# jhidalgocarrio/slam-localization

Hardware: NVIDIA B200
Metric: filter-steps/sec (predict+update) (higher is better)
Workload: dtype f64

## Files before the change

### slam-localization_b200/csrc/slb_api.cu

```cuda
#include <cstdio>
#include <cstdlib>
#include <cstring>
#include <atomic>
#include <new>

#include <dlfcn.h>
#include <nccl.h>

#include "slb_internal.h"
#include "slb_math.cuh"

namespace slb {

static thread_local char g_err[512] = "";
static std::atomic<int64_t> g_launches{0};

int set_error(int code, const char *what, cudaError_t ce) {
    if (ce != cudaSuccess)
        snprintf(g_err, sizeof(g_err), "%s: %s", what, cudaGetErrorString(ce));
    else
        snprintf(g_err, sizeof(g_err), "%s", what);
    return code;
}
void count_launch(int n) { g_launches.fetch_add(n, std::memory_order_relaxed); }
// ... 21 lines not shown
    const int c = e - r * (r + 1) / 2;
    soa[(size_t)e * stride + B0 + i] = dense[(size_t)i * N * N + r * N + c];
}
__global__ void soa_to_dense_P(const double *soa, double *dense, int B0, int cnt, int N, int stride) {
    const int64_t t = (int64_t)blockIdx.x * blockDim.x + threadIdx.x;
    if (t >= (int64_t)cnt * N * N) return;
    const int i = (int)(t / (N * N)), rc = (int)(t - (int64_t)i * N * N);
    int r = rc / N, c = rc - r * N;
    if (c > r) { const int x = r; r = c; c = x; }
    dense[t] = soa[(size_t)(r * (r + 1) / 2 + c) * stride + B0 + i];
}
__global__ void aos_to_rec_mu(const double *aos, double *rec, int B0, int cnt, int QD, int qstride) {
    const int t = blockIdx.x * blockDim.x + threadIdx.x;
    if (t >= cnt * QD) return;
    const int i = t / QD, c = t - i * QD;
    rec[(size_t)(B0 + i) * qstride + c] = aos[t];
}
__global__ void rec_to_aos_mu(const double *rec, double *aos, int B0, int cnt, int QD, int qstride, int off = 0) {
    const int t = blockIdx.x * blockDim.x + threadIdx.x;
    if (t >= cnt * QD) return;
    const int i = t / QD, c = t - i * QD;
    aos[t] = rec[(size_t)(B0 + i) * qstride + off + c];
}
__global__ void dense_to_rec_P(const double *dense, double *rec, int B0, int cnt, int N, int pstride) {
    const int64_t t = (int64_t)blockIdx.x * blockDim.x + threadIdx.x;
    if (t >= (int64_t)cnt * N * N) return;
    const int i = (int)(t / (N * N)), rc = (int)(t - (int64_t)i * N * N);
    const int r = rc / N, c = rc - r * N;
    if (c <= r) rec[(size_t)(B0 + i) * pstride + r * (r + 1) / 2 + c] = dense[t];
}
__global__ void rec_to_dense_P(const double *rec, double *dense, int B0, int cnt, int N, int pstride) {
    const int64_t t = (int64_t)blockIdx.x * blockDim.x + threadIdx.x;
    if (t >= (int64_t)cnt * N * N) return;
    const int i = (int)(t / (N * N)), rc = (int)(t - (int64_t)i * N * N);
    int r = rc / N, c = rc - r * N;
    if (c > r) { const int x = r; r = c; c = x; }
    dense[t] = rec[(size_t)(B0 + i) * pstride + r * (r + 1) / 2 + c];
}

__global__ void replicate_soa(double *a, int rows, int stride, int B, int count) {
    const int64_t t = (int64_t)blockIdx.x * blockDim.x + threadIdx.x;
    if (t >= (int64_t)rows * B) return;
    const int r = (int)(t / B), i = (int)(t - (int64_t)r * B);
    if (i >= count) a[(size_t)r * stride + i] = a[(size_t)r * stride + i % count];
}
__global__ void replicate_rec(double *a, int per, int B, int count) {
    const int64_t t = (int64_t)blockIdx.x * blockDim.x + threadIdx.x;
    if (t >= (int64_t)per * B) return;
    const int i = (int)(t / per), e = (int)(t - (int64_t)i * per);
    if (i >= count) a[(size_t)i * per + e] = a[(size_t)(i % count) * per + e];
}

__global__ void status_count(const int32_t *st, int B, unsigned long long *counts) {
    unsigned long long c[SLB_NSTATUS];
#pragma unroll
    for (int b = 0; b < SLB_NSTATUS; ++b) c[b] = 0;
    for (int i = blockIdx.x * blockDim.x + threadIdx.x; i < B; i += gridDim.x * blockDim.x) {
        const int s = st[i];
#pragma unroll
        for (int b = 0; b < SLB_NSTATUS; ++b) c[b] += (s >> b) & 1;
// ... 218 lines not shown
    if (!h || offset < 0 || count < 1 || offset + count > h->QD)
        return set_error(SLB_ERR_INVALID, "slb_set_output_slice: the slice must lie inside the q-vector");
    h->out_off = offset;
    h->out_len = count;
    return SLB_OK;
}
int slb_dof(slb_handle h) { return h ? h->N : SLB_ERR_INVALID; }
int slb_qdim(slb_handle h) { return h ? h->QD : SLB_ERR_INVALID; }

int slb_device_ptr(slb_handle h, int field, void **dev) {
    if (!h || !dev) return set_error(SLB_ERR_INVALID, "slb_device_ptr: null argument");
    switch (field) {
        case SLB_FIELD_MU: *dev = h->mu; return SLB_OK;
        case SLB_FIELD_P: *dev = h->P; return SLB_OK;
        case SLB_FIELD_STATUS: *dev = h->status; return SLB_OK;
        case SLB_FIELD_OUTLIERS: *dev = h->outliers; return SLB_OK;
    }
    return set_error(SLB_ERR_INVALID, "slb_device_ptr: unknown field");
}

static int transfer(slb_handle h, int field, void *host, size_t count, cudaStream_t s, bool up) {
    if (!h || !host) return set_error(SLB_ERR_INVALID, "slb_upload/download: null argument");
    DeviceGuard guard(h->cfg.device);
    const bool soa = h->cfg.kind == SLB_KIND_UKF;
    if (field == SLB_FIELD_STATUS || field == SLB_FIELD_OUTLIERS) {
        if (up) return set_error(SLB_ERR_INVALID, "slb_upload: status fields are read-only");
        if (count != (size_t)h->B) return set_error(SLB_ERR_INVALID, "slb_download: count must equal batch");
        SLB_CUDA(cudaMemcpyAsync(host, field == SLB_FIELD_STATUS ? h->status : h->outliers, (size_t)h->B * 4,
                                 cudaMemcpyDeviceToHost, s));
        SLB_CUDA(cudaStreamSynchronize(s));
        return SLB_OK;
    }
    size_t per;
    if (field == SLB_FIELD_MU) per = h->QD;
    else if (field == SLB_FIELD_P) per = (size_t)h->N * h->N;
    else return set_error(SLB_ERR_INVALID, "slb_upload/download: unknown field");
    if (count == 0 || count % per != 0 || count > per * h->B)
        return set_error(SLB_ERR_INVALID, "slb_upload/download: count must be k * per-instance size, 1 <= k <= batch");
    const int nin = (int)(count / per);
    const int chunk = (int)(h->stage_bytes / (per * 8));
    double *hp = (double *)host;
    for (int b0 = 0; b0 < nin; b0 += chunk) {
        const int cnt = (nin - b0) < chunk ? (nin - b0) : chunk;
        const size_t bytes = (size_t)cnt * per * 8;
        const int64_t work = (int64_t)cnt * (field == SLB_FIELD_MU ? h->QD : (up && soa ? h->NP : h->N * h->N));
        const int tpb = 256;
        const int grid = (int)((work + tpb - 1) / tpb);
        if (up) {
            SLB_CUDA(cudaMemcpyAsync(h->stage, hp + (size_t)b0 * per, bytes, cudaMemcpyHostToDevice, s));
            if (field == SLB_FIELD_MU) {
                if (soa) aos_to_soa_mu<<<grid, tpb, 0, s>>>(h->stage, h->mu, b0, cnt, h->QD, h->stride);
                else aos_to_rec_mu<<<grid, tpb, 0, s>>>(h->stage, h->mu, b0, cnt, h->QD, h->qstride);
            } else {
                if (soa) dense_to_soa_P<<<grid, tpb, 0, s>>>(h->stage, h->P, b0, cnt, h->N, h->stride);
                else dense_to_rec_P<<<grid, tpb, 0, s>>>(h->stage, h->P, b0, cnt, h->N, h->pstride);
            }
            count_launch();
            SLB_CUDA(cudaGetLastError());
        } else {
            if (field == SLB_FIELD_MU) {
                if (soa) soa_to_aos_mu<<<grid, tpb, 0, s>>>(h->mu, h->stage, b0, cnt, h->QD, h->stride);
                else rec_to_aos_mu<<<grid, tpb, 0, s>>>(h->mu, h->stage, b0, cnt, h->QD, h->qstride);
            } else {
                if (soa) soa_to_dense_P<<<grid, tpb, 0, s>>>(h->P, h->stage, b0, cnt, h->N, h->stride);
                else rec_to_dense_P<<<grid, tpb, 0, s>>>(h->P, h->stage, b0, cnt, h->N, h->pstride);
            }
            count_launch();
            SLB_CUDA(cudaGetLastError());
            SLB_CUDA(cudaMemcpyAsync(hp + (size_t)b0 * per, h->stage, bytes, cudaMemcpyDeviceToHost, s));
        }
        SLB_CUDA(cudaStreamSynchronize(s));
    }
    return SLB_OK;
}

int slb_upload(slb_handle h, int field, const void *host, size_t count, void *stream) {
    return transfer(h, field, const_cast<void *>(host), count, S(stream), true);
}
int slb_download(slb_handle h, int field, void *host, size_t count, void *stream) {
    return transfer(h, field, host, count, S(stream), false);
}

int slb_replicate(slb_handle h, int count, void *stream) {
    if (!h || count <= 0 || count > h->B) return set_error(SLB_ERR_INVALID, "slb_replicate: bad count");
    DeviceGuard guard(h->cfg.device);
    cudaStream_t s = S(stream);
    if (count == h->B) return SLB_OK;
    const int tpb = 256;
// ... 572 lines not shown
```

### slam-localization_b200/csrc/slb_check.cu

```cuda
#include "slb_internal.h"
#include "slb_math.cuh"

namespace slbd {

struct ChkLayout {
    int nblk;
    unsigned long long so3mask;
    int nfeat;
    int N, QD, NP, pstride, qstride;
};

SLB_DEV double warp_max(double v) {
#pragma unroll
    for (int o = 16; o > 0; o >>= 1) v = fmax(v, __shfl_xor_sync(0xffffffffu, v, o));
    return v;
}

__global__ void __launch_bounds__(32) check_sigma_points_kernel(const double *mu, const double *P, int B, ChkLayout l,
                                                                int32_t *flags, double *diff) {
    extern __shared__ double sm[];
    const int lane = threadIdx.x;
    const int N = l.N, QD = l.QD, NP = l.NP, NS = 2 * N + 1;
    double *Lp = sm, *Pa = Lp + NP, *D = Pa + NP, *mus = D + 32 * N, *ref = mus + QD, *md = ref + QD;
    for (int inst = blockIdx.x; inst < B; inst += gridDim.x) {
        const double *Pg = P + (size_t)inst * l.pstride, *mug = mu + (size_t)inst * l.qstride;
        __syncwarp();
        for (int e = lane; e < NP; e += 32) { Lp[e] = Pg[e]; Pa[e] = 0.0; }
        for (int e = lane; e < QD; e += 32) { mus[e] = mug[e]; ref[e] = mug[e]; }
        __syncwarp();
        bool ok = true;
        for (int k = 0; k < N && ok; ++k) {
            const double dkk = Lp[tri(k, k)];
            ok = dkk > 0.0;
            if (!ok) break;
            const double s = sqrt(dkk), inv = 1.0 / s;
            __syncwarp();
            for (int i = k + lane; i < N; i += 32) Lp[tri(i, k)] = i == k ? s : Lp[tri(i, k)] * inv;
            __syncwarp();
            for (int i = k + 1 + lane; i < N; i += 32) {
                const double lik = Lp[tri(i, k)];
                for (int j = k + 1; j <= i; ++j) Lp[tri(i, j)] = fma(-lik, Lp[tri(j, k)], Lp[tri(i, j)]);
            }
            __syncwarp();
        }
        if (!ok) {
            if (lane == 0) {
                flags[inst] = 4;
                if (diff) { diff[2 * (size_t)inst] = 0.0; diff[2 * (size_t)inst + 1] = 0.0; }
            }
            continue;
// ... 67 lines not shown
                        } else {
                            for (int c = 0; c < 3; ++c) ref[o + c] += md[3 * b + c];
                        }
                    }
                    o += so3 ? 4 : 3;
                }
                for (int f = lane; f < l.nfeat; f += 32) ref[o + f] += md[3 * l.nblk + f];
            }
            __syncwarp();
        } while (sqrt(nrm2) > 1e-6 && ++it < 10000);
        for (int s0 = 0; s0 < NS; s0 += 32) {
            __syncwarp();
            deviation(s0 + lane);
            __syncwarp();
            for (int i = 0; i < N; ++i)
                for (int j = lane; j <= i; j += 32) {
                    double a = 0.0;
                    for (int t = 0; t < 32; ++t) a = fma(D[t * N + i], D[t * N + j], a);
                    Pa[tri(i, j)] += 0.5 * a;
                }
        }
        __syncwarp();
        double dP = 0.0;
        for (int e = lane; e < NP; e += 32) dP = fmax(dP, fabs(Pa[e] - Pg[e]));
        dP = warp_max(dP);
        double dm = 0.0;
        {
            int o = 0;
            for (int b = 0; b < l.nblk; ++b) {
                const bool so3 = (l.so3mask >> b) & 1ull;
                if (b % 32 == lane) {
                    if (so3) {
                        const double q[4] = {mus[o], mus[o + 1], mus[o + 2], mus[o + 3]};
                        const double r[4] = {ref[o], ref[o + 1], ref[o + 2], ref[o + 3]};
                        double t[4], w[3];
                        quat_cmul(q, r, t);
                        so3_log(t, w);
                        for (int c = 0; c < 3; ++c) dm = fmax(dm, fabs(w[c]));
                    } else {
                        for (int c = 0; c < 3; ++c) dm = fmax(dm, fabs(ref[o + c] - mus[o + c]));
                    }
                }
                o += so3 ? 4 : 3;
            }
            for (int f = lane; f < l.nfeat; f += 32) dm = fmax(dm, fabs(ref[o + f] - mus[o + f]));
        }
        dm = warp_max(dm);
        if (lane == 0) {
            flags[inst] = (!(dP <= 1e-6) ? 1 : 0) | (!(dm <= 1e-12) ? 2 : 0);
            if (diff) { diff[2 * (size_t)inst] = dP; diff[2 * (size_t)inst + 1] = dm; }
        }
    }
}

}

namespace slb {

int launch_check_sigma_points(const slb_batch_s *h, int32_t *flags, double *diff, cudaStream_t s) {
    slbd::ChkLayout l;
    l.N = h->N; l.QD = h->QD; l.NP = h->NP; l.pstride = h->pstride; l.qstride = h->qstride;
    l.so3mask = 0;
    if (h->cfg.kind == SLB_KIND_USCKF) {
        l.nblk = 12; l.nfeat = h->cfg.nk + h->cfg.nl;
        l.so3mask = (1ull << 1) | (1ull << 5) | (1ull << 9);
    } else if (h->cfg.kind == SLB_KIND_MSCKF) {
        l.nblk = 4 + 2 * h->cfg.nclones; l.nfeat = 0;
        l.so3mask = 1ull << 1;
        for (int j = 0; j < h->cfg.nclones; ++j) l.so3mask |= 1ull << (4 + 2 * j + 1);
    } else {
        return set_error(SLB_ERR_INVALID, "slb_check_sigma_points: Usckf / Msckf batches only (the reference's ukfom::ukf has no checkSigmaPoints)");
    }
    const size_t smem = ((size_t)2 * l.NP + 32 * l.N + 2 * l.QD + l.N) * sizeof(double);
    SLB_CUDA(cudaFuncSetAttribute(slbd::check_sigma_points_kernel, cudaFuncAttributeMaxDynamicSharedMemorySize, (int)smem));
    int grid = h->B < 148 * 3 * 8 ? h->B : 148 * 3 * 8;
    slbd::check_sigma_points_kernel<<<grid, 32, smem, s>>>(h->mu, h->P, h->B, l, flags, diff);
    count_launch();
    SLB_CUDA(cudaGetLastError());
    return SLB_OK;
}

}
```

### slam-localization_b200/csrc/slb_math.cuh

```cuda
#pragma once
#include <cuda_runtime.h>
#include <stdint.h>

namespace slbd {

#define SLB_DEV __device__ __forceinline__
#define SLB_HD __host__ __device__ __forceinline__

template <int NB_, unsigned MASK_>
struct Layout {
    static constexpr int NB = NB_;
    static constexpr unsigned MASK = MASK_;
    static constexpr int N = 3 * NB_;
    static constexpr int NP = N * (N + 1) / 2;
    SLB_HD static constexpr bool so3(int b) { return (MASK_ >> b) & 1u; }
    SLB_HD static constexpr int qoff(int b) {
        int o = 0;
        for (int i = 0; i < b; ++i) o += ((MASK_ >> i) & 1u) ? 4 : 3;
        return o;
    }
    static constexpr int QD = qoff(NB_);
};
typedef Layout<2, 0x2> LayPose6;
typedef Layout<3, 0x2> LayMtk9;
typedef Layout<4, 0x2> LayState12;

SLB_HD constexpr int tri(int i, int j) { return i * (i + 1) / 2 + j; }

SLB_DEV double rcp_fast(double w) {
    double r;
    asm("rcp.approx.ftz.f64 %0, %1;" : "=d"(r) : "d"(w));
    double e = fma(-w, r, 1.0);
    r = fma(r, e, r);
    e = fma(-w, r, 1.0);
    r = fma(r, e, r);
    return r;
}
SLB_DEV void sqrt_rsqrt(double x, double &s, double &rs) {
    double y;
    asm("rsqrt.approx.ftz.f64 %0, %1;" : "=d"(y) : "d"(x));
    double e = fma(-(x * y), y, 1.0);
    y = fma(0.5 * y, e, y);
    e = fma(-(x * y), y, 1.0);
    y = fma(0.5 * y, e, y);
    double r = x * y;
    r = fma(fma(-r, r, x), 0.5 * y, r);
    s = r;
    rs = y;
}

// ... 167 lines not shown
```

### slam-localization_b200/csrc/slb_predict12.cuh

```cuda
#pragma once
#include "slb_internal.h"
#include "slb_models.cuh"

namespace slbd {

constexpr unsigned FULL = 0xffffffffu;
SLB_DEV double warp_sum(double v) {
#pragma unroll
    for (int o = 16; o > 0; o >>= 1) v += __shfl_xor_sync(FULL, v, o);
    return v;
}
SLB_DEV double bcast(double v, int src) { return __shfl_sync(FULL, v, src); }

template <int N_>
struct CycCfg {
    static constexpr int N = N_;
    static constexpr int RT = (N_ + 3) / 4;
    static constexpr int CT = (N_ + 7) / 8;
    SLB_HD static constexpr int cb(int k) { return k * N_ - k * (k - 1) / 2; }
    SLB_HD static constexpr bool exists(int r, int c) { return 4 * r < N_ && 8 * c < N_ && 4 * r + 3 >= 8 * c; }
    SLB_HD static constexpr bool live(int k, int r, int c) { return exists(r, c) && 8 * c + 7 > k && 4 * r + 3 > k; }
    SLB_HD static constexpr bool row_live(int k, int r) {
        for (int c = 0; c < CT; ++c)
            if (live(k, r, c)) return true;
// ... 60 lines not shown
}
SLB_DEV void bulk_g2s(void *dst, const void *src, unsigned bytes, uint64_t *bar) {
    asm volatile("cp.async.bulk.shared::cluster.global.mbarrier::complete_tx::bytes [%0], [%1], %2, [%3];\n" ::"r"(saddr(dst)),
                 "l"(src), "r"(bytes), "r"(saddr(bar))
                 : "memory");
}
SLB_DEV void mbar_wait(uint64_t *bar, unsigned parity) {
    unsigned done = 0;
    while (!done) {
        asm volatile(
            "{\n .reg .pred p;\n mbarrier.try_wait.parity.shared::cta.b64 p, [%1], %2;\n selp.u32 %0, 1, 0, p;\n}\n"
            : "=r"(done)
            : "r"(saddr(bar)), "r"(parity)
            : "memory");
    }
}

SLB_DEV void dmma884(double &d0, double &d1, double a, double b) {
    asm volatile("mma.sync.aligned.m8n8k4.row.col.f64.f64.f64.f64 {%0,%1}, {%2}, {%3}, {%0,%1};\n"
                 : "+d"(d0), "+d"(d1)
                 : "d"(a), "d"(b));
}

constexpr int PRED_PR = 366;
constexpr int PRED_PF = 28 * 12;
constexpr int PRED_DS = 20;
constexpr int PRED_LS = 78 + 16;
constexpr int PRED_SM = PRED_PR + PRED_PF + PRED_LS + 28 * PRED_DS + 144 + 12 * PRED_DS + 16 + 2;
static_assert(16 * PRED_SM * 8 <= 227 * 1024, "two CTAs of 8 warps per SM");
SLB_DEV void pred_cp_async8(double *smem_dst, const double *gsrc) {
    asm volatile("cp.async.ca.shared.global [%0], [%1], 8;\n" ::"r"(saddr(smem_dst)), "l"(gsrc) : "memory");
}
SLB_DEV void pred_cp_async_wait_all() { asm volatile("cp.async.commit_group;\n cp.async.wait_group 0;\n" ::: "memory"); }

template <int PM, int WPB, int ROW0, int MU0, bool CROSS>
__global__ void __launch_bounds__(WPB * 32, 2) predict12_kernel(slb::FilterArgs a) {
    typedef LayState12 L;
    typedef CycCfg<12> C;
    extern __shared__ __align__(16) double smem[];
    const int lane = threadIdx.x & 31, w = threadIdx.x >> 5;
    const int inst = blockIdx.x * WPB + w;
    if (inst >= a.B) return;
    double *Pr = smem + (size_t)w * PRED_SM, *Pf = Pr + PRED_PR, *Ls = Pf + PRED_PF, *D = Ls + PRED_LS, *W = D + 28 * PRED_DS,
           *Fk = W + 144, *rsd = Fk + 12 * PRED_DS;
    const int nf = CROSS ? a.nk + a.nl : 0;
    constexpr int T0 = ROW0 * (ROW0 + 1) / 2, T1 = (ROW0 + 12) * (ROW0 + 13) / 2, SPAN = T1 - T0;
    static_assert(SPAN <= PRED_PR, "row span");
    double *Pg = a.P + (size_t)inst * a.pstride;
    double *mug = a.mu + (size_t)inst * a.qstride;
    auto PR = [&](int r, int c) -> double & { return Pr[tri(ROW0 + r, c) - T0]; };
    const int a_ = lane & 3, b_ = lane >> 2;

    static_assert((T0 * 8) % 16 == 0 && (SPAN * 8) % 16 == 0 && PRED_SM % 2 == 0, "bulk copy needs 16-byte alignment");
    uint64_t *bar = reinterpret_cast<uint64_t *>(rsd + 16);
    if (lane == 0) {
        mbar_init(bar, 1);
        mbar_expect_tx(bar, SPAN * 8);
        bulk_g2s(Pr, Pg + T0, SPAN * 8, bar);
    }
    for (int e = lane; e < nf * 12; e += 32) {
        const int r = e / 12, c = e - r * 12;
        pred_cp_async8(Pf + e, Pg + tri(36 + r, 24 + c));
    }
    double mu[13];
#pragma unroll
    for (int c = 0; c < 13; ++c) mu[c] = mug[MU0 + c];
    ProcessModel<PM> f;
    {
        double u[ProcessModel<PM>::NU];
#pragma unroll
        for (int c = 0; c < ProcessModel<PM>::NU; ++c) u[c] = a.u[(size_t)inst * ProcessModel<PM>::NU + c];
        f.prepare(u, a.dt);
    }
    pred_cp_async_wait_all();
    __syncwarp();
    mbar_wait(bar, 0);

    double T[C::RT][C::CT];
#pragma unroll
    for (int r = 0; r < C::RT; ++r)
#pragma unroll
        for (int c = 0; c < C::CT; ++c)
            if (C::exists(r, c)) {
                const int i = a_ + 4 * r, j = b_ + 8 * c;
                T[r][c] = (i < 12 && j <= i) ? PR(i, ROW0 + j) : 0.0;
// ... 105 lines not shown
                for (int J = 0; J < 3; ++J) oc[I][J][0] = oc[I][J][1] = 0.0;
#pragma unroll
            for (int k0 = 0; k0 < 12; k0 += 4) {
                const double fa0 = Fk[r0 * PRED_DS + k0 + a_], fa1 = Fk[r1 * PRED_DS + k0 + a_];
#pragma unroll
                for (int J = 0; J < 3; ++J) {
                    const double bv = PR(k0 + a_, 8 * J + b_);
                    dmma884(oc[0][J][0], oc[0][J][1], fa0, bv);
                    dmma884(oc[1][J][0], oc[1][J][1], fa1, bv);
                }
            }
        }
        double of[4][2][2];
        const int nft = (nf + 7) >> 3;
        {
            const int c0 = min(b_, 11), c1 = min(8 + b_, 11);
#pragma unroll
            for (int I = 0; I < 4; ++I) {
                of[I][0][0] = of[I][0][1] = of[I][1][0] = of[I][1][1] = 0.0;
                if (I < nft) {
                    const int fr = min(8 * I + b_, nf - 1);
#pragma unroll
                    for (int k0 = 0; k0 < 12; k0 += 4) {
                        const double av = Pf[fr * 12 + k0 + a_];
                        dmma884(of[I][0][0], of[I][0][1], av, Fk[c0 * PRED_DS + k0 + a_]);
                        dmma884(of[I][1][0], of[I][1][1], av, Fk[c1 * PRED_DS + k0 + a_]);
                    }
                }
            }
        }
        __syncwarp();
#pragma unroll
        for (int I = 0; I < 2; ++I)
#pragma unroll
            for (int J = 0; J < 3; ++J) {
                const int r = 8 * I + b_, c = 8 * J + 2 * a_;
                if (r < 12) { PR(r, c) = oc[I][J][0]; PR(r, c + 1) = oc[I][J][1]; }
            }
#pragma unroll
        for (int I = 0; I < 4; ++I)
            if (I < nft) {
#pragma unroll
                for (int J = 0; J < 2; ++J) {
                    const int fr = 8 * I + b_, c = 8 * J + 2 * a_;
                    if (fr < nf && c < 12) { Pf[fr * 12 + c] = of[I][J][0]; Pf[fr * 12 + c + 1] = of[I][J][1]; }
                }
            }
        __syncwarp();
    } else {
        __syncwarp();
    }
    for (int e = lane; e < SPAN; e += 32) Pg[T0 + e] = Pr[e];
    for (int e = lane; e < nf * 12; e += 32) {
        const int r = e / 12, c = e - r * 12;
        Pg[tri(36 + r, 24 + c)] = Pf[e];
    }
    bool finite = true;
#pragma unroll
    for (int c = 0; c < 13; ++c) {
        finite = finite && isfinite(ref[c]);
        if (lane == c) mug[MU0 + c] = ref[c];
    }
    if (!finite) st |= SLB_ST_NONFINITE;
    if (st && lane == 0) a.status[inst] |= st;
}

}
```

### slam-localization_b200/csrc/slb_usckf.cu

```cuda
#include <cstdlib>

#include "slb_predict12.cuh"
#include "slb_usckf_step.cuh"

namespace slbd {

__global__ void usckf_clone_kernel(slb::FilterArgs a, int mode) {
    const int64_t t = (int64_t)blockIdx.x * blockDim.x + threadIdx.x;
    const int per = 13 + 12 * 12 * 2;
    if (t >= (int64_t)a.B * per) return;
    const int inst = (int)(t / per), e = (int)(t - (int64_t)inst * per);
    double *P = a.P + (size_t)inst * a.pstride, *mu = a.mu + (size_t)inst * a.qstride;
    auto sym = [&](int r, int c) { return r >= c ? P[tri(r, c)] : P[tri(c, r)]; };
    if (e < 13) {
        if (mode == SLB_STATEK_I) mu[13 + e] = mu[26 + e];
        else mu[e] = mu[13 + e];
        return;
    }
    const int q = e - 13, blk = q / 144, rc = q - blk * 144, r = rc / 12, c = rc - r * 12;
    if (mode == SLB_STATEK_I) {
        if (blk == 0) {
            const double v = sym(24 + r, 24 + c);
            if (c <= r) P[tri(12 + r, 12 + c)] = v;
            P[tri(24 + r, 12 + c)] = v;
        } else {
            P[tri(24 + r, c)] = 0.0;
            P[tri(12 + r, c)] = 0.0;
        }
    } else if (blk == 0) {
        const double v = sym(12 + r, 12 + c);
        if (c <= r) P[tri(r, c)] = v;
        P[tri(12 + r, c)] = v;
    }
}

__global__ void usckf_set_measurement_kernel(slb::FilterArgs a, int mode) {
    const int N = 36 + a.nk + a.nl, NP = N * (N + 1) / 2;
    const int nfe = NP - 666;
    const int per = nfe + (mode == SLB_STATEK ? a.nk : a.nl);
    const int64_t t = (int64_t)blockIdx.x * blockDim.x + threadIdx.x;
    if (t >= (int64_t)a.B * per) return;
    const int inst = (int)(t / per), e = (int)(t - (int64_t)inst * per);
    double *P = a.P + (size_t)inst * a.pstride, *mu = a.mu + (size_t)inst * a.qstride;
    const int len = mode == SLB_STATEK ? a.nk : a.nl;
    const int f0 = mode == SLB_STATEK ? 0 : a.nk;
    if (e >= nfe) {
        const int c = e - nfe;
        mu[39 + f0 + c] = a.z[(size_t)inst * len + c];
        return;
    }
    int r = 36;
    while (tri(r + 1, 0) - 666 <= e) ++r;
    const int c = e - (tri(r, 0) - 666);
    const int fr = r - 36, fc = c - 36;
    double v = 0.0;
    if (c >= 36) {
        const bool rin = fr >= f0 && fr < f0 + len, cin = fc >= f0 && fc < f0 + len;
        if (rin && cin) v = a.R[(fr - f0) * len + (fc - f0)];
        else if (!rin && !cin) v = P[tri(r, c)];
    }
    P[tri(r, c)] = v;
}

}

namespace slb {

template <int PM>
static int launch_predict_t(const FilterArgs &a, cudaStream_t s) {
    constexpr int WPB = 8;
    constexpr size_t smem = (size_t)WPB * slbd::PRED_SM * sizeof(double);
    auto kern = slbd::predict12_kernel<PM, WPB, 24, 26, true>;
    SLB_CUDA(cudaFuncSetAttribute(kern, cudaFuncAttributeMaxDynamicSharedMemorySize, (int)smem));
    kern<<<(a.B + WPB - 1) / WPB, WPB * 32, smem, s>>>(a);
    count_launch();
    SLB_CUDA(cudaGetLastError());
    return SLB_OK;
}

#define SLB_USCKF_SHAPES(X) X(3, 0) X(3, 3) X(3, 6) X(3, 9) X(6, 0) X(6, 3) X(6, 6) X(9, 0) X(9, 3)
bool usckf_shape_supported(int nk, int nl) {
#define SLB_USCKF_SHAPE(NK_, NL_) \
    if (nk == NK_ && nl == NL_) return true;
    SLB_USCKF_SHAPES(SLB_USCKF_SHAPE)
#undef SLB_USCKF_SHAPE
    return false;
}

template <int NK, int NL, bool PRED, bool UPD>
static int launch_step_t(const FilterArgs &a, cudaStream_t s) {
    typedef slbd::StepCfg<NK, NL> C;
    constexpr size_t pw = (size_t)C::SM * sizeof(double);
    constexpr size_t SM_BYTES = 228 * 1024, CTA_MAX = 227 * 1024, RSV = 1024;
#ifdef SLB_USCKF_WPB
    constexpr int WPB = SLB_USCKF_WPB;
#else
    constexpr int WPB = 2 * (6 * pw + RSV) <= SM_BYTES ? 6 : 4;
#endif
    constexpr size_t smem = (size_t)WPB * pw;
    constexpr int fit = (int)(SM_BYTES / (smem + RSV));
    constexpr int cap = 12 / WPB < 1 ? 1 : 12 / WPB;
    constexpr int MINB = fit > cap ? cap : fit < 1 ? 1 : fit;
    auto kern = slbd::usckf_step_kernel<SLB_PM_USCKF_TEST, NK, NL, PRED, UPD, WPB, MINB>;
// ... 32 lines not shown
#define SLB_USCKF_SHAPE(NK_, NL_) \
    if (a.nk == NK_ && a.nl == NL_) return launch_step_nknl<NK_, NL_>(predict, a, s);
        SLB_USCKF_SHAPES(SLB_USCKF_SHAPE)
#undef SLB_USCKF_SHAPE
        return set_error(SLB_ERR_INVALID, "usckf update: (nk, nl) is not one of the built shapes (see slb_usckf_shape_supported)");
    }
    return SLB_OK;
}

int launch_usckf_clone(int mode, const FilterArgs &a, cudaStream_t s) {
    if (mode != SLB_STATEK_I && mode != SLB_STATEK_L) return SLB_OK;
    const int64_t work = (int64_t)a.B * (13 + 288);
    slbd::usckf_clone_kernel<<<(unsigned)((work + 255) / 256), 256, 0, s>>>(a, mode);
    count_launch();
    SLB_CUDA(cudaGetLastError());
    return SLB_OK;
}

int launch_usckf_set_measurement(int mode, const FilterArgs &a, cudaStream_t s) {
    if (mode != SLB_STATEK && mode != SLB_STATEK_L) return SLB_OK;
    const int N = 36 + a.nk + a.nl;
    const int len = mode == SLB_STATEK ? a.nk : a.nl;
    if (len == 0) return SLB_OK;
    const int64_t work = (int64_t)a.B * (N * (N + 1) / 2 - 666 + len);
    slbd::usckf_set_measurement_kernel<<<(unsigned)((work + 255) / 256), 256, 0, s>>>(a, mode);
    count_launch();
    SLB_CUDA(cudaGetLastError());
    return SLB_OK;
}

}
```

### slam-localization_b200/csrc/slb_usckf_step.cuh

```cuda
#pragma once
#include "slb_predict12.cuh"

#ifndef SLB_USCKF_CTA_SYNC
#define SLB_USCKF_CTA_SYNC 0
#endif
#if SLB_USCKF_CTA_SYNC
#define SLB_CTA_SYNC() __syncthreads()
#else
#define SLB_CTA_SYNC() ((void)0)
#endif

namespace slbd {

template <int NK_, int NL_>
struct StepCfg {
    static constexpr int NK = NK_, NL = NL_, NF = NK_ + NL_;
    static constexpr int N = 36 + NK_ + NL_;
    static constexpr int NP = N * (N + 1) / 2;
    static constexpr int PSTR = (NP + 15) / 16 * 16;
    static constexpr int QD = 39 + NK_ + NL_;
    static constexpr int QS = (QD + 1) / 2 * 2;
    static constexpr int NT = (N + 7) / 8;
    static constexpr int NPAD = 8 * NT;
    static constexpr int JM = 36 + NK_;
// ... 302 lines not shown
            sigma_group<C, (P >> 2)>(s, mus, Lf, Wg, dv, lane);
            SLB_CTA_SYNC();
        }
        PanelStep<C, P + 1>::run(s, mus, Lf, Lraw, Wg, dv, lane);
    }
};
template <class C>
struct PanelStep<C, C::NPAN> {
    SLB_DEV static void run(UpdState<C> &, const double *, double *, double *, double *, double *, int) {}
};

template <int NK, int NL>
SLB_DEV int usckf_update_smem(double *Ps, double *mus, double *scr, const double *zs, const slb::FilterArgs &a, int lane,
                              bool &dirty) {
    typedef StepCfg<NK, NL> C;
    constexpr int N = C::N, NT = C::NT, NPAD = C::NPAD, JLAST = C::JLAST, KP = C::KP;
    const int a_ = lane & 3, b_ = lane >> 2;
    double *Lf = scr, *Lraw = scr + C::LF, *Ks = scr, *Cs = scr + NPAD * KP, *Wg = scr + C::SCR0, *dv = Wg + C::WGS,
           *dl = Cs + NPAD * KP;
    UpdState<C> s;
    s.ok = true;
    auto elem = [&](int i, int j) -> double {
        if (i >= N || j >= N) return i == j ? 1.0 : 0.0;
        return i >= j ? Ps[tri(i, j)] : Ps[tri(j, i)];
    };
#pragma unroll
    for (int I = 0; I < NT; ++I)
#pragma unroll
        for (int J = 0; J <= JLAST; ++J)
            if (J <= I) {
                const int i = 8 * I + b_, j = 8 * J + 2 * a_;
                s.c0[I][J] = elem(i, j);
                s.c1[I][J] = elem(i, j + 1);
            }
#pragma unroll
    for (int c = 0; c < NK; ++c) s.px0[c] = s.px1[c] = s.esum[c] = 0.0;
#pragma unroll
    for (int e = 0; e < NK * (NK + 1) / 2; ++e) s.eep[e] = 0.0;
    {
        double pk[3], qk[4], pi[3], qi[4], ft[NK];
#pragma unroll
        for (int c = 0; c < 3; ++c) { pk[c] = mus[c]; pi[c] = mus[26 + c]; }
#pragma unroll
        for (int c = 0; c < 4; ++c) { qk[c] = mus[3 + c]; qi[c] = mus[29 + c]; }
#pragma unroll
        for (int c = 0; c < NK; ++c) ft[c] = mus[39 + c];
        vo_model<NK>(pk, qk, pi, qi, ft, s.z0);
    }
    PanelStep<C, 0>::run(s, mus, Lf, Lraw, Wg, dv, lane);
    if (!s.ok) return SLB_ST_CHOL_FAIL;

    constexpr double NS = (double)(2 * N + 1);
    double ebar[NK], S[NK * (NK + 1) / 2];
// ... 78 lines not shown
                finite = finite && isfinite(o);
            }
        }
    }
    for (int f = lane; f < NK + NL; f += 32) {
        const double o = mus[39 + f] + dl[36 + f];
        mus[39 + f] = o;
        finite = finite && isfinite(o);
    }
    {
        double fa[NT][KP / 4], fb[NT][KP / 4];
#pragma unroll
        for (int I = 0; I < NT; ++I)
#pragma unroll
            for (int kk = 0; kk < KP / 4; ++kk) {
                fa[I][kk] = Cs[(8 * I + b_) * KP + 4 * kk + a_];
                fb[I][kk] = Ks[(8 * I + b_) * KP + 4 * kk + a_];
            }
#pragma unroll
        for (int I = 0; I < NT; ++I)
#pragma unroll
            for (int J = 0; J <= I; ++J) {
                const int i = 8 * I + b_, j = 8 * J + 2 * a_;
                const bool w0 = i < N && j <= i, w1 = i < N && j + 1 <= i;
                double p0 = w0 ? Ps[tri(i, j)] : 0.0, p1 = w1 ? Ps[tri(i, j + 1)] : 0.0;
#pragma unroll
                for (int kk = 0; kk < KP / 4; ++kk) dmma884(p0, p1, fa[I][kk], fb[J][kk]);
                if (w0) Ps[tri(i, j)] = p0;
                if (w1) Ps[tri(i, j + 1)] = p1;
            }
    }
    return __all_sync(FULL, finite) ? 0 : SLB_ST_NONFINITE;
}

template <int PM, int NF>
SLB_DEV int usckf_predict_smem(double *Ps, double *mus, double *scr, const double *u, double dt, const double *Qg, int lane,
                               bool &dirty) {
    typedef LayState12 L;
    typedef CycCfg<12> C;
    constexpr int ROW0 = 24, MU0 = 26;
    double *Ls = scr, *D = Ls + PRED_LS, *W = D + 28 * PRED_DS, *Fk = W + 144, *rsd = Fk + 12 * PRED_DS, *slots = rsd + 16;
    auto PR = [&](int r, int c) -> double & { return Ps[tri(ROW0 + r, c)]; };
    auto PF = [&](int fr, int c) -> double & { return Ps[tri(36 + fr, 24 + c)]; };
    const int a_ = lane & 3, b_ = lane >> 2;
    double mu[13];
#pragma unroll
    for (int c = 0; c < 13; ++c) mu[c] = mus[MU0 + c];
    ProcessModel<PM> f;
    f.prepare(u, dt);
    double T[C::RT][C::CT];
#pragma unroll
    for (int r = 0; r < C::RT; ++r)
#pragma unroll
        for (int c = 0; c < C::CT; ++c)
            if (C::exists(r, c)) {
                const int i = a_ + 4 * r, j = b_ + 8 * c;
                T[r][c] = (i < 12 && j <= i) ? PR(i, ROW0 + j) : 0.0;
            }
    bool ok = true;
    {
        const double x0 = __shfl_sync(FULL, T[0][0], 0);
        CholStep<C, 0>::run(T, Ls, a_, b_, ok, x0, -rcp_fast(x0));
    }
    if (!ok) return SLB_ST_CHOL_FAIL;
    __syncwarp();
    if (lane < 12) {
// ... 102 lines not shown
            }
        }
    }
    constexpr int NFT = (NF + 7) / 8;
    double of[NFT > 0 ? NFT : 1][2][2];
    {
        const int c0 = min(b_, 11), c1 = min(8 + b_, 11);
#pragma unroll
        for (int I = 0; I < NFT; ++I) {
            of[I][0][0] = of[I][0][1] = of[I][1][0] = of[I][1][1] = 0.0;
            const int fr = min(8 * I + b_, NF - 1);
#pragma unroll
            for (int k0 = 0; k0 < 12; k0 += 4) {
                const double av = PF(fr, k0 + a_);
                dmma884(of[I][0][0], of[I][0][1], av, Fk[c0 * PRED_DS + k0 + a_]);
                dmma884(of[I][1][0], of[I][1][1], av, Fk[c1 * PRED_DS + k0 + a_]);
            }
        }
    }
    __syncwarp();
#pragma unroll
    for (int I = 0; I < 2; ++I)
#pragma unroll
        for (int J = 0; J < 3; ++J) {
            const int r = 8 * I + b_, c = 8 * J + 2 * a_;
            if (r < 12) { PR(r, c) = oc[I][J][0]; PR(r, c + 1) = oc[I][J][1]; }
        }
#pragma unroll
    for (int I = 0; I < NFT; ++I) {
#pragma unroll
        for (int J = 0; J < 2; ++J) {
            const int fr = 8 * I + b_, c = 8 * J + 2 * a_;
            if (fr < NF && c < 12) { PF(fr, c) = of[I][J][0]; PF(fr, c + 1) = of[I][J][1]; }
        }
    }
    bool finite = true;
#pragma unroll
    for (int c = 0; c < 13; ++c) {
        finite = finite && isfinite(ref[c]);
        if (lane == c) mus[MU0 + c] = ref[c];
    }
    if (!finite) st |= SLB_ST_NONFINITE;
    __syncwarp();
    return st;
}

template <int PM, int NK, int NL, bool PRED, bool UPD, int WPB, int MINB>
__global__ void __launch_bounds__(WPB * 32, MINB) usckf_step_kernel(slb::FilterArgs a) {
    typedef StepCfg<NK, NL> C;
    extern __shared__ __align__(128) double smem[];
// ... 49 lines not shown
```

Baseline: 92.20 million.

## Store USCKF covariance in 8x8 tile-major packed layout for vectorized MMA fragment access

Introduces a tiled packed-triangular record layout (prec) for USCKF covariances, where off-diagonal 8x8 tiles are stored contiguously in the MMA fragment order. Fragment loads and stores in the update and predict paths become single double2 accesses per lane instead of scattered triangular indexing. The aim is lower shared-memory instruction count and fewer bank conflicts in the hot DMMA loops. Upload/download, the checker, the state-clone and measurement kernels, and the predict staging buffers are all adapted to the new layout, which adds index arithmetic and complexity to these paths.

```diff
diff --git a/slam-localization_b200/csrc/slb_api.cu b/slam-localization_b200/csrc/slb_api.cu
--- a/slam-localization_b200/csrc/slb_api.cu
+++ b/slam-localization_b200/csrc/slb_api.cu
@@ -67,20 +67,20 @@
     const int i = t / QD, c = t - i * QD;
     aos[t] = rec[(size_t)(B0 + i) * qstride + off + c];
 }
-__global__ void dense_to_rec_P(const double *dense, double *rec, int B0, int cnt, int N, int pstride) {
+__global__ void dense_to_rec_P(const double *dense, double *rec, int B0, int cnt, int N, int pstride, bool tiled) {
     const int64_t t = (int64_t)blockIdx.x * blockDim.x + threadIdx.x;
     if (t >= (int64_t)cnt * N * N) return;
     const int i = (int)(t / (N * N)), rc = (int)(t - (int64_t)i * N * N);
     const int r = rc / N, c = rc - r * N;
-    if (c <= r) rec[(size_t)(B0 + i) * pstride + r * (r + 1) / 2 + c] = dense[t];
-}
-__global__ void rec_to_dense_P(const double *rec, double *dense, int B0, int cnt, int N, int pstride) {
+    if (c <= r) rec[(size_t)(B0 + i) * pstride + (tiled ? slbd::prec(N, r, c) : slbd::tri(r, c))] = dense[t];
+}
+__global__ void rec_to_dense_P(const double *rec, double *dense, int B0, int cnt, int N, int pstride, bool tiled) {
     const int64_t t = (int64_t)blockIdx.x * blockDim.x + threadIdx.x;
     if (t >= (int64_t)cnt * N * N) return;
     const int i = (int)(t / (N * N)), rc = (int)(t - (int64_t)i * N * N);
     int r = rc / N, c = rc - r * N;
     if (c > r) { const int x = r; r = c; c = x; }
-    dense[t] = rec[(size_t)(B0 + i) * pstride + r * (r + 1) / 2 + c];
+    dense[t] = rec[(size_t)(B0 + i) * pstride + (tiled ? slbd::prec(N, r, c) : slbd::tri(r, c))];
 }
 
 __global__ void replicate_soa(double *a, int rows, int stride, int B, int count) {
@@ -345,7 +345,7 @@
 static int transfer(slb_handle h, int field, void *host, size_t count, cudaStream_t s, bool up) {
     if (!h || !host) return set_error(SLB_ERR_INVALID, "slb_upload/download: null argument");
     DeviceGuard guard(h->cfg.device);
-    const bool soa = h->cfg.kind == SLB_KIND_UKF;
+    const bool soa = h->cfg.kind == SLB_KIND_UKF, tiled = h->cfg.kind == SLB_KIND_USCKF;
     if (field == SLB_FIELD_STATUS || field == SLB_FIELD_OUTLIERS) {
         if (up) return set_error(SLB_ERR_INVALID, "slb_upload: status fields are read-only");
         if (count != (size_t)h->B) return set_error(SLB_ERR_INVALID, "slb_download: count must equal batch");
@@ -376,7 +376,7 @@
                 else aos_to_rec_mu<<<grid, tpb, 0, s>>>(h->stage, h->mu, b0, cnt, h->QD, h->qstride);
             } else {
                 if (soa) dense_to_soa_P<<<grid, tpb, 0, s>>>(h->stage, h->P, b0, cnt, h->N, h->stride);
-                else dense_to_rec_P<<<grid, tpb, 0, s>>>(h->stage, h->P, b0, cnt, h->N, h->pstride);
+                else dense_to_rec_P<<<grid, tpb, 0, s>>>(h->stage, h->P, b0, cnt, h->N, h->pstride, tiled);
             }
             count_launch();
             SLB_CUDA(cudaGetLastError());
@@ -386,7 +386,7 @@
                 else rec_to_aos_mu<<<grid, tpb, 0, s>>>(h->mu, h->stage, b0, cnt, h->QD, h->qstride);
             } else {
                 if (soa) soa_to_dense_P<<<grid, tpb, 0, s>>>(h->P, h->stage, b0, cnt, h->N, h->stride);
-                else rec_to_dense_P<<<grid, tpb, 0, s>>>(h->P, h->stage, b0, cnt, h->N, h->pstride);
+                else rec_to_dense_P<<<grid, tpb, 0, s>>>(h->P, h->stage, b0, cnt, h->N, h->pstride, tiled);
             }
             count_launch();
             SLB_CUDA(cudaGetLastError());
diff --git a/slam-localization_b200/csrc/slb_check.cu b/slam-localization_b200/csrc/slb_check.cu
--- a/slam-localization_b200/csrc/slb_check.cu
+++ b/slam-localization_b200/csrc/slb_check.cu
@@ -8,6 +8,7 @@
     unsigned long long so3mask;
     int nfeat;
     int N, QD, NP, pstride, qstride;
+    int tiled;
 };
 
 SLB_DEV double warp_max(double v) {
@@ -24,8 +25,10 @@
     double *Lp = sm, *Pa = Lp + NP, *D = Pa + NP, *mus = D + 32 * N, *ref = mus + QD, *md = ref + QD;
     for (int inst = blockIdx.x; inst < B; inst += gridDim.x) {
         const double *Pg = P + (size_t)inst * l.pstride, *mug = mu + (size_t)inst * l.qstride;
+        auto rec = [&](int i, int j) { return l.tiled ? prec(N, i, j) : tri(i, j); };
         __syncwarp();
-        for (int e = lane; e < NP; e += 32) { Lp[e] = Pg[e]; Pa[e] = 0.0; }
+        for (int i = 0; i < N; ++i)
+            for (int j = lane; j <= i; j += 32) { Lp[tri(i, j)] = Pg[rec(i, j)]; Pa[tri(i, j)] = 0.0; }
         for (int e = lane; e < QD; e += 32) { mus[e] = mug[e]; ref[e] = mug[e]; }
         __syncwarp();
         bool ok = true;
@@ -139,7 +142,8 @@
         }
         __syncwarp();
         double dP = 0.0;
-        for (int e = lane; e < NP; e += 32) dP = fmax(dP, fabs(Pa[e] - Pg[e]));
+        for (int i = 0; i < N; ++i)
+            for (int j = lane; j <= i; j += 32) dP = fmax(dP, fabs(Pa[tri(i, j)] - Pg[rec(i, j)]));
         dP = warp_max(dP);
         double dm = 0.0;
         {
@@ -178,6 +182,7 @@
     slbd::ChkLayout l;
     l.N = h->N; l.QD = h->QD; l.NP = h->NP; l.pstride = h->pstride; l.qstride = h->qstride;
     l.so3mask = 0;
+    l.tiled = h->cfg.kind == SLB_KIND_USCKF;
     if (h->cfg.kind == SLB_KIND_USCKF) {
         l.nblk = 12; l.nfeat = h->cfg.nk + h->cfg.nl;
         l.so3mask = (1ull << 1) | (1ull << 5) | (1ull << 9);
diff --git a/slam-localization_b200/csrc/slb_math.cuh b/slam-localization_b200/csrc/slb_math.cuh
--- a/slam-localization_b200/csrc/slb_math.cuh
+++ b/slam-localization_b200/csrc/slb_math.cuh
@@ -26,6 +26,11 @@
 typedef Layout<4, 0x2> LayState12;
 
 SLB_HD constexpr int tri(int i, int j) { return i * (i + 1) / 2 + j; }
+
+SLB_HD constexpr int prec(int N, int i, int j) {
+    const int I = i >> 3, J = j >> 3, h = N - 8 * I < 8 ? N - 8 * I : 8;
+    return tri(8 * I, 0) + 8 * h * J + (J < I ? 8 * (i & 7) + (j & 7) : tri(i & 7, j & 7));
+}
 
 SLB_DEV double rcp_fast(double w) {
     double r;
diff --git a/slam-localization_b200/csrc/slb_predict12.cuh b/slam-localization_b200/csrc/slb_predict12.cuh
--- a/slam-localization_b200/csrc/slb_predict12.cuh
+++ b/slam-localization_b200/csrc/slb_predict12.cuh
@@ -106,8 +106,8 @@
                  : "d"(a), "d"(b));
 }
 
-constexpr int PRED_PR = 366;
-constexpr int PRED_PF = 28 * 12;
+constexpr int PRED_PR = 520;
+constexpr int PRED_PF = 8 * 12;
 constexpr int PRED_DS = 20;
 constexpr int PRED_LS = 78 + 16;
 constexpr int PRED_SM = PRED_PR + PRED_PF + PRED_LS + 28 * PRED_DS + 144 + 12 * PRED_DS + 16 + 2;
@@ -127,24 +127,36 @@
     if (inst >= a.B) return;
     double *Pr = smem + (size_t)w * PRED_SM, *Pf = Pr + PRED_PR, *Ls = Pf + PRED_PF, *D = Ls + PRED_LS, *W = D + 28 * PRED_DS,
            *Fk = W + 144, *rsd = Fk + 12 * PRED_DS;
-    const int nf = CROSS ? a.nk + a.nl : 0;
-    constexpr int T0 = ROW0 * (ROW0 + 1) / 2, T1 = (ROW0 + 12) * (ROW0 + 13) / 2, SPAN = T1 - T0;
-    static_assert(SPAN <= PRED_PR, "row span");
+    static_assert(!CROSS || ROW0 == 24, "the tiled span is tile rows 3..4");
+    const int nf = CROSS ? a.nk + a.nl : 0, N = CROSS ? 36 + nf : ROW0 + 12;
+    constexpr int T0 = ROW0 * (ROW0 + 1) / 2, T1 = (ROW0 + 12) * (ROW0 + 13) / 2;
+    constexpr int RS = CROSS ? 40 : ROW0 + 12;
+    constexpr int NFS = RS - 36;
+    const int SPAN = CROSS ? tri(min(N, RS), 0) - T0 : T1 - T0;
+    const int nfr = CROSS && nf > NFS ? nf - NFS : 0;
+    static_assert(tri(RS, 0) - T0 <= PRED_PR && (!CROSS || 12 * (48 - RS) <= PRED_PF), "row span");
     double *Pg = a.P + (size_t)inst * a.pstride;
     double *mug = a.mu + (size_t)inst * a.qstride;
-    auto PR = [&](int r, int c) -> double & { return Pr[tri(ROW0 + r, c) - T0]; };
+    auto PR = [&](int r, int c) -> double & {
+        return Pr[(CROSS ? prec(N, ROW0 + r, c) : tri(ROW0 + r, c)) - T0];
+    };
+    auto PF = [&](int fr, int c) -> double & {
+        return fr < NFS ? PR(12 + fr, 24 + c) : Pf[(fr - NFS) * 12 + c];
+    };
     const int a_ = lane & 3, b_ = lane >> 2;
 
-    static_assert((T0 * 8) % 16 == 0 && (SPAN * 8) % 16 == 0 && PRED_SM % 2 == 0, "bulk copy needs 16-byte alignment");
+    static_assert((T0 * 8) % 16 == 0 && ((T1 - T0) * 8) % 16 == 0 && PRED_SM % 2 == 0 &&
+                      (!CROSS || (((tri(RS, 0) - T0) * 8) % 16 == 0 && ((tri(39, 0) - T0) * 8) % 16 == 0)),
+                  "bulk copy needs 16-byte alignment");
     uint64_t *bar = reinterpret_cast<uint64_t *>(rsd + 16);
     if (lane == 0) {
         mbar_init(bar, 1);
         mbar_expect_tx(bar, SPAN * 8);
         bulk_g2s(Pr, Pg + T0, SPAN * 8, bar);
     }
-    for (int e = lane; e < nf * 12; e += 32) {
+    for (int e = lane; e < nfr * 12; e += 32) {
         const int r = e / 12, c = e - r * 12;
-        pred_cp_async8(Pf + e, Pg + tri(36 + r, 24 + c));
+        pred_cp_async8(Pf + e, Pg + prec(N, RS + r, 24 + c));
     }
     double mu[13];
 #pragma unroll
@@ -296,7 +308,7 @@
                     const int fr = min(8 * I + b_, nf - 1);
 #pragma unroll
                     for (int k0 = 0; k0 < 12; k0 += 4) {
-                        const double av = Pf[fr * 12 + k0 + a_];
+                        const double av = PF(fr, k0 + a_);
                         dmma884(of[I][0][0], of[I][0][1], av, Fk[c0 * PRED_DS + k0 + a_]);
                         dmma884(of[I][1][0], of[I][1][1], av, Fk[c1 * PRED_DS + k0 + a_]);
                     }
@@ -307,17 +319,17 @@
 #pragma unroll
         for (int I = 0; I < 2; ++I)
 #pragma unroll
-            for (int J = 0; J < 3; ++J) {
-                const int r = 8 * I + b_, c = 8 * J + 2 * a_;
-                if (r < 12) { PR(r, c) = oc[I][J][0]; PR(r, c + 1) = oc[I][J][1]; }
-            }
+            for (int J = 0; J < 3; ++J)
+                if (8 * I + b_ < 12)
+                    *reinterpret_cast<double2 *>(Pr + prec(N, ROW0 + 8 * I, 8 * J) - T0 + 2 * lane) =
+                        make_double2(oc[I][J][0], oc[I][J][1]);
 #pragma unroll
         for (int I = 0; I < 4; ++I)
             if (I < nft) {
 #pragma unroll
                 for (int J = 0; J < 2; ++J) {
                     const int fr = 8 * I + b_, c = 8 * J + 2 * a_;
-                    if (fr < nf && c < 12) { Pf[fr * 12 + c] = of[I][J][0]; Pf[fr * 12 + c + 1] = of[I][J][1]; }
+                    if (fr < nf && c < 12) { PF(fr, c) = of[I][J][0]; PF(fr, c + 1) = of[I][J][1]; }
                 }
             }
         __syncwarp();
@@ -325,9 +337,9 @@
         __syncwarp();
     }
     for (int e = lane; e < SPAN; e += 32) Pg[T0 + e] = Pr[e];
-    for (int e = lane; e < nf * 12; e += 32) {
+    for (int e = lane; e < nfr * 12; e += 32) {
         const int r = e / 12, c = e - r * 12;
-        Pg[tri(36 + r, 24 + c)] = Pf[e];
+        Pg[prec(N, RS + r, 24 + c)] = Pf[e];
     }
     bool finite = true;
 #pragma unroll
diff --git a/slam-localization_b200/csrc/slb_usckf.cu b/slam-localization_b200/csrc/slb_usckf.cu
--- a/slam-localization_b200/csrc/slb_usckf.cu
+++ b/slam-localization_b200/csrc/slb_usckf.cu
@@ -11,7 +11,9 @@
     if (t >= (int64_t)a.B * per) return;
     const int inst = (int)(t / per), e = (int)(t - (int64_t)inst * per);
     double *P = a.P + (size_t)inst * a.pstride, *mu = a.mu + (size_t)inst * a.qstride;
-    auto sym = [&](int r, int c) { return r >= c ? P[tri(r, c)] : P[tri(c, r)]; };
+    const int N = 36 + a.nk + a.nl;
+    auto at = [&](int r, int c) -> double & { return P[prec(N, r, c)]; };
+    auto sym = [&](int r, int c) { return r >= c ? at(r, c) : at(c, r); };
     if (e < 13) {
         if (mode == SLB_STATEK_I) mu[13 + e] = mu[26 + e];
         else mu[e] = mu[13 + e];
@@ -21,22 +23,22 @@
     if (mode == SLB_STATEK_I) {
         if (blk == 0) {
             const double v = sym(24 + r, 24 + c);
-            if (c <= r) P[tri(12 + r, 12 + c)] = v;
-            P[tri(24 + r, 12 + c)] = v;
+            if (c <= r) at(12 + r, 12 + c) = v;
+            at(24 + r, 12 + c) = v;
         } else {
-            P[tri(24 + r, c)] = 0.0;
-            P[tri(12 + r, c)] = 0.0;
+            at(24 + r, c) = 0.0;
+            at(12 + r, c) = 0.0;
         }
     } else if (blk == 0) {
         const double v = sym(12 + r, 12 + c);
-        if (c <= r) P[tri(r, c)] = v;
-        P[tri(12 + r, c)] = v;
+        if (c <= r) at(r, c) = v;
+        at(12 + r, c) = v;
     }
 }
 
 __global__ void usckf_set_measurement_kernel(slb::FilterArgs a, int mode) {
-    const int N = 36 + a.nk + a.nl, NP = N * (N + 1) / 2;
-    const int nfe = NP - 666;
+    const int N = 36 + a.nk + a.nl;
+    const int nfe = (N - 36) * N;
     const int per = nfe + (mode == SLB_STATEK ? a.nk : a.nl);
     const int64_t t = (int64_t)blockIdx.x * blockDim.x + threadIdx.x;
     if (t >= (int64_t)a.B * per) return;
@@ -49,17 +51,16 @@
         mu[39 + f0 + c] = a.z[(size_t)inst * len + c];
         return;
     }
-    int r = 36;
-    while (tri(r + 1, 0) - 666 <= e) ++r;
-    const int c = e - (tri(r, 0) - 666);
+    const int r = 36 + e / N, c = e - (r - 36) * N;
+    if (c > r) return;
     const int fr = r - 36, fc = c - 36;
     double v = 0.0;
     if (c >= 36) {
         const bool rin = fr >= f0 && fr < f0 + len, cin = fc >= f0 && fc < f0 + len;
         if (rin && cin) v = a.R[(fr - f0) * len + (fc - f0)];
-        else if (!rin && !cin) v = P[tri(r, c)];
+        else if (!rin && !cin) v = P[prec(N, r, c)];
     }
-    P[tri(r, c)] = v;
+    P[prec(N, r, c)] = v;
 }
 
 }
@@ -79,6 +80,21 @@
 }
 
 #define SLB_USCKF_SHAPES(X) X(3, 0) X(3, 3) X(3, 6) X(3, 9) X(6, 0) X(6, 3) X(6, 6) X(9, 0) X(9, 3)
+static constexpr bool prec_fills_record(int N) {
+    bool seen[48 * 49 / 2] = {};
+    for (int i = 0; i < N; ++i)
+        for (int j = 0; j <= i; ++j) {
+            const int o = slbd::prec(N, i, j);
+            if (o < 0 || o >= N * (N + 1) / 2 || seen[o]) return false;
+            if ((j & 7) == 0 && (j >> 3) < (i >> 3) && o % 2 != 0) return false;
+            seen[o] = true;
+        }
+    return true;
+}
+#define SLB_USCKF_SHAPE(NK_, NL_) static_assert(prec_fills_record(36 + NK_ + NL_), "USCKF record layout");
+SLB_USCKF_SHAPES(SLB_USCKF_SHAPE)
+#undef SLB_USCKF_SHAPE
+
 bool usckf_shape_supported(int nk, int nl) {
 #define SLB_USCKF_SHAPE(NK_, NL_) \
     if (nk == NK_ && nl == NL_) return true;
@@ -157,7 +173,7 @@
     const int N = 36 + a.nk + a.nl;
     const int len = mode == SLB_STATEK ? a.nk : a.nl;
     if (len == 0) return SLB_OK;
-    const int64_t work = (int64_t)a.B * (N * (N + 1) / 2 - 666 + len);
+    const int64_t work = (int64_t)a.B * ((N - 36) * N + len);
     slbd::usckf_set_measurement_kernel<<<(unsigned)((work + 255) / 256), 256, 0, s>>>(a, mode);
     count_launch();
     SLB_CUDA(cudaGetLastError());
diff --git a/slam-localization_b200/csrc/slb_usckf_step.cuh b/slam-localization_b200/csrc/slb_usckf_step.cuh
--- a/slam-localization_b200/csrc/slb_usckf_step.cuh
+++ b/slam-localization_b200/csrc/slb_usckf_step.cuh
@@ -348,13 +348,18 @@
     s.ok = true;
     auto elem = [&](int i, int j) -> double {
         if (i >= N || j >= N) return i == j ? 1.0 : 0.0;
-        return i >= j ? Ps[tri(i, j)] : Ps[tri(j, i)];
+        return i >= j ? Ps[prec(N, i, j)] : Ps[prec(N, j, i)];
     };
 #pragma unroll
     for (int I = 0; I < NT; ++I)
 #pragma unroll
         for (int J = 0; J <= JLAST; ++J)
-            if (J <= I) {
+            if (J < I) {
+                double2 v = make_double2(0.0, 0.0);
+                if (8 * I + b_ < N) v = *reinterpret_cast<const double2 *>(Ps + prec(N, 8 * I, 8 * J) + 2 * lane);
+                s.c0[I][J] = v.x;
+                s.c1[I][J] = v.y;
+            } else if (J == I) {
                 const int i = 8 * I + b_, j = 8 * J + 2 * a_;
                 s.c0[I][J] = elem(i, j);
                 s.c1[I][J] = elem(i, j + 1);
@@ -479,12 +484,21 @@
 #pragma unroll
             for (int J = 0; J <= I; ++J) {
                 const int i = 8 * I + b_, j = 8 * J + 2 * a_;
-                const bool w0 = i < N && j <= i, w1 = i < N && j + 1 <= i;
-                double p0 = w0 ? Ps[tri(i, j)] : 0.0, p1 = w1 ? Ps[tri(i, j + 1)] : 0.0;
-#pragma unroll
-                for (int kk = 0; kk < KP / 4; ++kk) dmma884(p0, p1, fa[I][kk], fb[J][kk]);
-                if (w0) Ps[tri(i, j)] = p0;
-                if (w1) Ps[tri(i, j + 1)] = p1;
+                if (J < I) {
+                    double2 *pp = reinterpret_cast<double2 *>(Ps + prec(N, 8 * I, 8 * J) + 2 * lane);
+                    const bool w = i < N;
+                    double2 p = w ? *pp : make_double2(0.0, 0.0);
+#pragma unroll
+                    for (int kk = 0; kk < KP / 4; ++kk) dmma884(p.x, p.y, fa[I][kk], fb[J][kk]);
+                    if (w) *pp = p;
+                } else {
+                    const bool w0 = i < N && j <= i, w1 = i < N && j + 1 <= i;
+                    double p0 = w0 ? Ps[prec(N, i, j)] : 0.0, p1 = w1 ? Ps[prec(N, i, j + 1)] : 0.0;
+#pragma unroll
+                    for (int kk = 0; kk < KP / 4; ++kk) dmma884(p0, p1, fa[I][kk], fb[J][kk]);
+                    if (w0) Ps[prec(N, i, j)] = p0;
+                    if (w1) Ps[prec(N, i, j + 1)] = p1;
+                }
             }
     }
     return __all_sync(FULL, finite) ? 0 : SLB_ST_NONFINITE;
@@ -495,10 +509,10 @@
                                bool &dirty) {
     typedef LayState12 L;
     typedef CycCfg<12> C;
-    constexpr int ROW0 = 24, MU0 = 26;
+    constexpr int ROW0 = 24, MU0 = 26, N = 36 + NF;
     double *Ls = scr, *D = Ls + PRED_LS, *W = D + 28 * PRED_DS, *Fk = W + 144, *rsd = Fk + 12 * PRED_DS, *slots = rsd + 16;
-    auto PR = [&](int r, int c) -> double & { return Ps[tri(ROW0 + r, c)]; };
-    auto PF = [&](int fr, int c) -> double & { return Ps[tri(36 + fr, 24 + c)]; };
+    auto PR = [&](int r, int c) -> double & { return Ps[prec(N, ROW0 + r, c)]; };
+    auto PF = [&](int fr, int c) -> double & { return Ps[prec(N, 36 + fr, 24 + c)]; };
     const int a_ = lane & 3, b_ = lane >> 2;
     double mu[13];
 #pragma unroll
@@ -647,10 +661,9 @@
 #pragma unroll
     for (int I = 0; I < 2; ++I)
 #pragma unroll
-        for (int J = 0; J < 3; ++J) {
-            const int r = 8 * I + b_, c = 8 * J + 2 * a_;
-            if (r < 12) { PR(r, c) = oc[I][J][0]; PR(r, c + 1) = oc[I][J][1]; }
-        }
+        for (int J = 0; J < 3; ++J)
+            if (8 * I + b_ < 12)
+                *reinterpret_cast<double2 *>(Ps + prec(N, ROW0 + 8 * I, 8 * J) + 2 * lane) = make_double2(oc[I][J][0], oc[I][J][1]);
 #pragma unroll
     for (int I = 0; I < NFT; ++I) {
 #pragma unroll
```

New measurement: 97.44 million, median of 6. 1.06x the previous value.
